# zhazorken/beom

Measured on AMD Instinct MI355X. Metric: cell-layer updates/s, higher is better.
Workload: dtype f64

## Files before the change

### beom_amd/csrc/beom_engine.hip

```cpp
#include <hip/hip_runtime.h>

#include <cmath>
#include <cstdarg>
#include <cstdio>
#include <cstdlib>
#include <cstring>
#include <algorithm>
#include <string>
#include <utility>
#include <vector>

#include "beom_dev.h"
#include "beom_kernels.h"
#include "beom_integrals.h"
#include "beom_series.h"
#include "beom_tracers.h"
#include "beom_tracers_lim.h"
#include "beom_floats.h"
#include "beom_moments.h"
#include "beom_tracer_moments.h"
#include "beom_dense_host.h"

namespace {

// ... 65 lines not shown
    ++A.count;
    ++A.launches;
}

struct beom_engine {
    beom_params P;
    int device = 0;
    hipStream_t stream = nullptr;
    hipStream_t own_stream = nullptr;
    StepTimer *timer = nullptr;
    DevView d{};
    bool dense = false;
    std::vector<void *> allocs;
    const int32_t *slot_of_dev = nullptr;
    bool embedded = false;
    void *stage = nullptr;
    size_t stage_bytes = 0;
    dim3 grid_cells0, grid_cells_layers_flat;
    bool wind = false, bot = false, top = false;
    bool fold_stress = true, fold_static_ok = false;
    bool up_tt = false, up_tb = false, up_tu = false;
    bool last_folded = false;
    bool last_uv_fused = false;
    float *h0r4_dev = nullptr, *out4[3] = {nullptr, nullptr, nullptr};
    float *diag4[3] = {nullptr, nullptr, nullptr};
    double *scan_dev = nullptr;
    int any_u = 0, any_v = 0;
    long long uniform_waves = 0, total_waves = 0;
    bool obc = false;
    bool obc_set = false;
    bool fuse = true;
    bool fuse_uv = true;
    bool lean_visc = true;
    bool visc_all_zero = true;
    bool lean_d2h = true;
    std::vector<int32_t> subc_host, neig_host, dev_index;
    bool lid = false, lid_ready = false;
    int lid_dstep = 2, lid_nring = 0, lid_maxwidth = 1;
    double *lid_ring = nullptr;
    unsigned long long *lid_maxd = nullptr;
    long long lid_sweeps = 0, lid_solves = 0, lid_launches = 0;
    int lid_last = 0;
    int profile_stride = 1;
    bool profile_rotate = false;
    bool split_prod = false;
    bool tile4 = false;
    bool mont_history = true;
    bool mont_keep = false;
    int mont_levels_valid = 0;
    bool hist_stale = false;
    bool last_mont_hist = false;
    bool plain_sweeps = true;
    int last_plain = 0;
    double *integ_part = nullptr, *integ_rows = nullptr;
    int integ_count = 0;
    int32_t *integ_cellmap = nullptr;
    int integ_xper = 0, integ_yper = 0;
    int ntrc = 0;
    int trc_scheme = 1;
    double *trc_q = nullptr, *trc_q_alt = nullptr, *trc_rq[2] = {nullptr, nullptr}, *trc_ctrg = nullptr;
    std::vector<void *> trc_allocs;
    long long nflt = 0;
    bool flt_ready = false;
    double *flt_x = nullptr, *flt_y = nullptr, *flt_k1x = nullptr, *flt_k1y = nullptr, *flt_xs = nullptr, *flt_ys = nullptr;
    int32_t *flt_layer = nullptr, *flt_rej = nullptr;
    unsigned long long *flt_first_dry = nullptr;
    double *flt_rec = nullptr;
    int flt_nrec = 0, flt_stride = 1;
    std::vector<int> flt_rec_tstp;
    long long flt_launches = 0;
    bool cellmap_known = false;
    std::vector<void *> flt_allocs;
    bool flt_band = false;
    FloatBand flt_fb{};
    unsigned long long *flt_in_s = nullptr, *flt_in_n = nullptr;
    int flt_xper = 0, flt_yper = 0;
    double flt_fmm = 0.0;
    long long flt_handovers = 0;
    Accum mom{&kFieldMoments};
    bool mom_by_caller = false;
    int last_tstp = 0;
    Accum tmom{&kTracerMoments};
    int ser_level = 0, ser_stride = 1, ser_nrec = 0, ser_jlo = 1, ser_rows = 0;
    bool ser_by_caller = false;
    double *ser_rec = nullptr;
    std::vector<int> ser_tstp;
    std::vector<void *> ser_allocs;
    char last_err[512] = {0};
};
static int hist_sync(beom_engine *E);
static int leave_mont_history(beom_engine *E);

namespace {

template <class T>
int alloc_plain(beom_engine *E, std::vector<void *> &owner, T **p, size_t n, char *errm, int errm_len, bool zero = true) {
    void *q = nullptr;
    HIP_TRY(hipMalloc(&q, n * sizeof(T)));
    owner.push_back(q);
    if (zero) HIP_TRY(hipMemsetAsync(q, 0, n * sizeof(T), E->stream));
    *p = (T *)q;
    return 0;
}
constexpr size_t kLead = 15;
template <class T>
int alloc_aligned(beom_engine *E, std::vector<void *> &owner, T **p, size_t n, char *errm, int errm_len, bool zero = true) {
// ... 612 lines not shown
    E->ser_tstp.push_back(tstp);
}
template <class CTX>
static bool launch_mont_all(beom_engine *E) {
    const dim3 g = CTX::grid(E->d, 1), b(BEOM_BLOCK);
    switch (E->d.nlay) {
#define CASE_NL(n) case n: hipLaunchKernelGGL((k_update_mont_all<CTX, n>), g, b, 0, E->stream, E->d); return true;
        CASE_NL(1) CASE_NL(2) CASE_NL(3) CASE_NL(4) CASE_NL(5) CASE_NL(6) CASE_NL(7) CASE_NL(8)
#undef CASE_NL
        default: return false;
    }
}
static void launch_mont(beom_engine *E, int ilay) {
    if (ilay == 0) {
        if (E->dense ? launch_mont_all<CellDense>(E) : launch_mont_all<CellGather>(E)) return;
    }
    const int nz = ilay ? 1 : E->d.nlay;
    LAUNCH_CTX(k_update_mont<CellGather>, k_update_mont<CellDense>, nz, E->d, ilay);
}
static bool biharm_tiled(const beom_engine *E) { return E->dense && E->P.svis > 0.0; }
static void launch_visc(beom_engine *E, int ilay) {
    const int nz = ilay ? 1 : E->d.nlay;
    LAUNCH_CTX(k_update_visc<CellGather>, k_update_visc<CellDense>, nz, E->d, ilay);
    if (E->d.svis > 0.0 && biharm_tiled(E) && ilay == 0) {
        if (E->tile4) hipLaunchKernelGGL(k_biharm_tiled<1>, biharm_tiled_grid<1>(E->d), dim3(BEOM_BLOCK), 0, E->stream, E->d);
        else hipLaunchKernelGGL(k_biharm_tiled<2>, biharm_tiled_grid<2>(E->d), dim3(BEOM_BLOCK), 0, E->stream, E->d);
    } else if (E->d.svis > 0.0) {
        const dim3 g = ilay ? E->grid_cells0 : E->grid_cells_layers_flat;
        hipLaunchKernelGGL(k_biharm_lap, g, dim3(BEOM_BLOCK), 0, E->stream, E->d, ilay);
        hipLaunchKernelGGL(k_biharm_flux, g, dim3(BEOM_BLOCK), 0, E->stream, E->d, ilay);
    }
}
template <bool XDIR>
static void launch_uv(beom_engine *E, int ilay, double gene, double ramp, double ctim, bool prod = false) {
    const int nz = ilay ? 1 : E->d.nlay;
    const int copy_hist = ilay ? 1 : 0;
    if (prod) hipLaunchKernelGGL((k_update_uv<CellDense, XDIR, true>), CellDense::grid(E->d, nz), dim3(BEOM_BLOCK), 0, E->stream, E->d, ilay, gene, ramp, ctim, copy_hist);
    else LAUNCH_CTX((k_update_uv<CellGather, XDIR>), (k_update_uv<CellDense, XDIR>), nz, E->d, ilay, gene, ramp, ctim, copy_hist);
    if (!copy_hist) { if (XDIR) rot3(E->d.dmx); else rot3(E->d.dmy); }
}
template <int Q>
static bool raw_mont_visc(beom_engine *E, bool leith, bool plain) {
    const dim3 g = mont_visc_grid<Q>(E->d), b(BEOM_BLOCK);
    switch (E->d.nlay) {
#define MV_GO(n, le, pl) hipLaunchKernelGGL((k_mont_visc<Q, n, le, pl>), g, b, 0, E->stream, E->d)
#define CASE_NL(n) case n: if (plain) { if (leith) MV_GO(n, true, true); else MV_GO(n, false, true); } \
                           else if (leith) MV_GO(n, true, false); else MV_GO(n, false, false); return true;
        CASE_NL(1) CASE_NL(2) CASE_NL(3) CASE_NL(4) CASE_NL(5) CASE_NL(6) CASE_NL(7) CASE_NL(8)
#undef CASE_NL
#undef MV_GO
        default: return false;
    }
}
template <int Q>
static void raw_uv_fused(beom_engine *E, bool first_x, bool prod, bool zv, bool hm, bool plain, double gene, double ramp, double ctim) {
    const dim3 g = uv_fused_grid<Q>(E->d), b(TileGeom<Q>::BLOCK);
    DevView &d = E->d;
#define UV_GO(kern, fx, pr, z) hipLaunchKernelGGL((kern<Q, fx, pr, z>), g, b, 0, E->stream, d, gene, ramp, ctim)
#define UV_PLAIN(fx, z, h) hipLaunchKernelGGL((k_uv_fused<Q, fx, true, z, h, true>), g, b, 0, E->stream, d, gene, ramp, ctim)
#define UV_PICK(fx) do { \
        if (plain) { if (hm) { if (zv) UV_PLAIN(fx, true, true); else UV_PLAIN(fx, false, true); } \
                     else { if (zv) UV_PLAIN(fx, true, false); else UV_PLAIN(fx, false, false); } } \
        else if (hm) { if (zv) hipLaunchKernelGGL((k_uv_fused<Q, fx, true, true, true>), g, b, 0, E->stream, d, gene, ramp, ctim); \
                       else hipLaunchKernelGGL((k_uv_fused<Q, fx, true, false, true>), g, b, 0, E->stream, d, gene, ramp, ctim); } \
        else if (d.stress_fold) { if (zv) UV_GO(k_uv_fused_sf, fx, true, true); else if (prod) UV_GO(k_uv_fused_sf, fx, true, false); else UV_GO(k_uv_fused_sf, fx, false, false); } \
        else { if (zv) UV_GO(k_uv_fused, fx, true, true); else if (prod) UV_GO(k_uv_fused, fx, true, false); else UV_GO(k_uv_fused, fx, false, false); } \
    } while (0)
    if (first_x) UV_PICK(true); else UV_PICK(false);
#undef UV_PICK
#undef UV_PLAIN
#undef UV_GO
}
static bool launch_mont_visc(beom_engine *E, bool uv_fused_follows, bool leith, bool keep_visc) {
    E->d.lean_d2h = uv_fused_follows && E->lean_d2h && !E->d.keep_diag;
    E->d.keep_visc = keep_visc;
    E->d.zero_visc = !leith && uv_fused_follows && E->lean_visc && E->visc_all_zero && E->P.dvis == 0.0 && E->P.bvis == 0.0 &&
                     !E->d.keep_diag;
    const bool plain = E->plain_sweeps && E->d.ocrp == 0.0 && !(E->d.rgld >= 0.5) && !E->d.has_hto && !E->d.keep_diag && !E->d.keep_visc;
    const bool ok = E->tile4 ? raw_mont_visc<1>(E, leith, plain) : raw_mont_visc<2>(E, leith, plain);
    if (ok && plain) E->last_plain |= 2;
    return ok;
}
static void uv_fused_swap(beom_engine *E, bool first_x, bool hm = false) {
    DevView &d = E->d;
    swp(d.u, d.u_alt); swp(d.v, d.v_alt);
    if (first_x) swp(d.h_v, d.hv_alt); else swp(d.h_u, d.hu_alt);
    if (hm) { E->hist_stale = true; return; }
    if (first_x) { rot4(d.dmx); rot3(d.dmy); }
    else         { rot4(d.dmy); rot3(d.dmx); }
}
static void launch_uv_fused(beom_engine *E, bool first_x, bool prod, double gene, double ramp, double ctim,
                            bool swap = true, bool hm = false) {
    const bool zv = prod && E->d.zero_visc;
    const DevView &d = E->d;
    const bool plain = E->plain_sweeps && prod && !d.stress_fold && !d.has_nudg && !d.has_tide && !d.has_stress && !d.has_bodf &&
                       !(d.rgld >= 0.5) && d.svis == 0.0;
    if (plain) E->last_plain |= 1;
    if (E->tile4) raw_uv_fused<1>(E, first_x, prod, zv, hm, plain, gene, ramp, ctim);
    else raw_uv_fused<2>(E, first_x, prod, zv, hm, plain, gene, ramp, ctim);
    if (swap) uv_fused_swap(E, first_x, hm);
}
static bool can_fuse(const beom_engine *E, int n_3d, bool first3) {
    const int nl = E->d.nlay;
    if (!(E->dense && E->fuse && nl <= 8) || E->P.svis > 0.0) return false;
    (void)n_3d;
    if (E->P.dvis > 1.e-3) return true;
    return !first3;
}
static void launch_lid_fluxes(beom_engine *E, bool first3) {
    if (first3) { launch_rebuild(E); return; }
    const dim3 g((unsigned)((E->d.ncell + BEOM_BLOCK - 1) / BEOM_BLOCK), (unsigned)E->d.nlay, 1);
    hipLaunchKernelGGL(k_rgld_upstream_fluxes, g, dim3(BEOM_BLOCK), 0, E->stream, E->d);
}
static void launch_lid_h_epilogue(beom_engine *E) {
    hipLaunchKernelGGL(k_rgld_h_epilogue, dim3((unsigned)((E->d.ncell + BEOM_BLOCK - 1) / BEOM_BLOCK)), dim3(BEOM_BLOCK), 0, E->stream, E->d);
}
static int lid_solve(beom_engine *E) {
    DevView &d = E->d;
    const int maxiters = 1000;
    const double pi_tol = 1.e-5;
    const int R = E->lid_nring, D = E->lid_dstep, nlev = d.sor_ndiag;
    const size_t bytes = (size_t)d.n1 * sizeof(double);
    if (hipMemcpyAsync(E->lid_ring, d.pi_s, bytes, hipMemcpyDeviceToDevice, E->stream) != hipSuccess) return -1;
    int s0 = 1, batch = std::min(R - 1, std::max(16, E->lid_last * 5 / 4 + 8)), chosen = 0;
    unsigned long long maxd[kLidBatch];
    while (!chosen) {
        const int nb = std::min(batch, maxiters - s0 + 1);
        if (hipMemsetAsync(E->lid_maxd, 0, nb * sizeof(unsigned long long), E->stream) != hipSuccess) return -1;
        const dim3 g((unsigned)((E->lid_maxwidth + BEOM_BLOCK - 1) / BEOM_BLOCK), (unsigned)nb, 1);
        const int tend = nlev - 1 + (nb - 1) * D;
        for (int t = 0; t <= tend; ++t)
            hipLaunchKernelGGL(k_rgld_gs_front, g, dim3(BEOM_BLOCK), 0, E->stream, d, E->lid_ring, R, s0, t, D, E->lid_maxd);
        E->lid_launches += tend + 1;
// ... 64 lines not shown
    s.fused_uv = E->dense && E->fuse_uv;
    return s;
}

static bool stress_folds(const beom_engine *E, const StepScalars &s) {
    return E->fold_stress && E->fold_static_ok && s.fused_uv && s.stress && !s.first3 && s.n_3d == 1 && !E->d.keep_diag &&
           (E->wind || !E->up_tt) && (E->bot || !E->up_tb) && (E->top || !E->up_tu);
}

static StepTimer *begin_step(beom_engine *E, int tstp, const StepScalars &s) {
    StepTimer *T = (E->timer && tstp % E->timer->stride == 0) ? E->timer : nullptr;
    if (T) { T->st = E->stream; T->step(tstp); }
    E->d.stress_fold = stress_folds(E, s) ? 1 : 0;
    E->last_folded = E->d.stress_fold != 0;
    return T;
}
template <class F>
static void timed(StepTimer *T, int c, F &&f) {
    if (T) T->begin(c);
    f();
    if (T) T->end();
}

static bool step_front(beom_engine *E, const StepScalars &s, StepTimer *T) {
    if (s.stress && !E->d.stress_fold) launch_stress(E);
    if (E->lid) launch_lid_fluxes(E, s.first3);
    else if (s.first3) launch_rebuild(E);
    if (E->ntrc > 0) timed(T, 7, [&] { launch_tracers(E, s.gene, s.ramp, s.ctim); });
    timed(T, 0, [&] {
        launch_h(E, s.gene, s.ramp, s.ctim);
        if (E->lid) launch_lid_h_epilogue(E);
    });
    const bool leith = E->P.dvis > 1.e-3 && s.upst;
    bool prod = false;
    timed(T, s.fused ? 5 : 1, [&] {
        prod = s.fused && launch_mont_visc(E, s.fused_uv, leith, leith && s.n_3d > 1);
        if (!prod) launch_mont(E, 0);
    });
    if (!prod && (s.first3 || leith || E->P.svis > 0.0)) timed(T, 2, [&] { launch_visc(E, 0); });
    return prod;
}

static bool mont_hist_step(const beom_engine *E, const StepScalars &s) {
    return E->mont_history && E->mont_keep && s.fused && s.fused_uv && s.gene != 0.0 && !stress_folds(E, s) &&
           E->mont_levels_valid >= 3;
}

static void one_step(beom_engine *E, int tstp, const StepScalars &s, int flt = -1) {
    if (flt >= 0 && (flt & 1)) launch_floats(E, 1, nullptr);
    const bool hm = mont_hist_step(E, s);
    if (!hm) (void)hist_sync(E);
    rotate_mont(E);
    StepTimer *T = begin_step(E, tstp, s);
    E->last_plain = 0;
    const bool prod = step_front(E, s, T);
    const bool u_first = tstp % 2 == 0;
    E->last_uv_fused = s.fused_uv;
    E->last_mont_hist = hm;
    if (E->mont_keep) E->mont_levels_valid = std::min(E->mont_levels_valid + 1, 3);
    if (s.fused_uv) timed(T, 6, [&] { launch_uv_fused(E, u_first, prod, s.gene, s.ramp, s.ctim, true, hm && prod); });
    else
        for (const bool x : {u_first, !u_first})
            timed(T, x ? 3 : 4, [&] {
                if (x) launch_uv<true>(E, 0, s.gene, s.ramp, s.ctim, prod);
                else launch_uv<false>(E, 0, s.gene, s.ramp, s.ctim, prod);
            });
    if (E->obc) {
        const dim3 g((unsigned)((E->d.nseg + BEOM_BLOCK - 1) / BEOM_BLOCK), (unsigned)E->d.nlay, 1);
        hipLaunchKernelGGL(k_no_gradient_obc, g, dim3(BEOM_BLOCK), 0, E->stream, E->d, 0);
        hipLaunchKernelGGL(k_no_gradient_obc, g, dim3(BEOM_BLOCK), 0, E->stream, E->d, 1);
    }
    if (E->lid) { launch_lid_fluxes(E, s.first3); launch_lid_pressure(E); }
    E->d.stress_fold = 0;
    if (flt >= 0) launch_floats_after(E, tstp, !(flt & 2));
    E->last_tstp = tstp;
    if (!E->mom_by_caller && accum_due(E->mom, tstp)) launch_moments(E, tstp);
    if (!E->mom_by_caller && accum_due(E->tmom, tstp)) launch_tracer_moments(E, tstp);
    if (!E->ser_by_caller && series_due(E, tstp)) launch_series(E, tstp);
}

template <bool PACK>
static int rows_copy(beom_handle E, int jlo, int nrows, void *dbuf, int jlo2, void *dbuf2) {
    if (!E || !dbuf || jlo < 1 || nrows < 1 || jlo + nrows - 1 > E->d.M) return -3;
    if (dbuf2 && (jlo2 < 1 || jlo2 + nrows - 1 > E->d.M)) return -3;
    if (hipSetDevice(E->device) != hipSuccess) return -9;
    const long long total = 5ll * E->d.nlay * nrows * E->d.L;
    hipLaunchKernelGGL((k_rows_copy<PACK>), dim3((unsigned)((total + BEOM_BLOCK - 1) / BEOM_BLOCK), dbuf2 ? 2u : 1u), dim3(BEOM_BLOCK),
                       0, E->stream, E->d, jlo, nrows, (double *)dbuf, jlo2, (double *)dbuf2);
    if (E->ntrc > 0) {
        const long long tq = (long long)E->ntrc * E->d.nlay * nrows * E->d.L;
        hipLaunchKernelGGL((k_rows_copy_q<PACK>), dim3((unsigned)((tq + BEOM_BLOCK - 1) / BEOM_BLOCK), dbuf2 ? 2u : 1u), dim3(BEOM_BLOCK),
                           0, E->stream, E->d, E->trc_q, E->ntrc, jlo, nrows, (double *)dbuf + total, jlo2, dbuf2 ? (double *)dbuf2 + total : nullptr);
    }
    return hipGetLastError() == hipSuccess ? 0 : -10;
}
extern "C" {

int beom_step(beom_handle E, int tstp_first, int nsteps, double tres, double dtd8, double dt_r,
              double rsta, int n_3d, char *errm, int errm_len) {
    if (!E) { set_err(errm, errm_len, "null handle"); return -1; }
    if (tstp_first < 1 || nsteps < 0 || n_3d < 1) { set_err(errm, errm_len, "beom_step: bad arguments"); return -3; }
    if (E->P.flag_nudging && E->P.mcbc < 0.5 && !E->obc && !E->obc_set) { set_err(errm, errm_len, "beom_step: mcbc = 0 with nudging needs beom_set_open_boundaries (no_gradient_obc, private_mod.f95:2613-2679)"); return -6; }
    if (E->lid && !E->lid_ready) { set_err(errm, errm_len, "beom_step: rgld = 1 needs beom_set_rigid_lid (the Poisson operators Ow, Os, Osum_ and the lid pressure, private_mod.f95:505-563)"); return -6; }
    const bool flt = E->nflt > 0 && !E->flt_band;
    if (flt && !E->flt_ready) { set_err(errm, errm_len, "beom_step: the handle's %lld floats have no positions yet (beom_upload_floats)", E->nflt); return -3; }
    if (flt && E->flt_nrec > 0) {
        long long due = 0;
// ... 38 lines not shown
int beom_profile_stop(beom_handle E, double *ms, int *launches, char *errm, int errm_len) {
    if (!E || !ms || !launches) { set_err(errm, errm_len, "null argument"); return -1; }
    if (!E->timer) { set_err(errm, errm_len, "beom_profile_stop without beom_profile_start"); return -3; }
    HIP_TRY(hipSetDevice(E->device));
    HIP_TRY(hipStreamSynchronize(E->stream));
    StepTimer &T = *E->timer;
    for (int c = 0; c < 8; ++c) { ms[c] = 0.0; launches[c] = 0; }
    for (size_t k = 0; k < T.cls.size(); ++k) {
        float t = 0.f;
        (void)hipEventElapsedTime(&t, T.ev[2 * k], T.ev[2 * k + 1]);
        ms[T.cls[k]] += (double)t;
        launches[T.cls[k]] += 1;
    }
    for (hipEvent_t ev : T.ev) (void)hipEventDestroy(ev);
    delete E->timer;
    E->timer = nullptr;
    HIP_TRY(hipGetLastError());
    return 0;
}

int beom_profile_steps(beom_handle E, int tstp_first, int nsteps, double tres, double dtd8, double dt_r,
                       double rsta, int n_3d, double *ms, int *launches, char *errm, int errm_len) {
    int rc = beom_profile_start(E);
    if (rc) { set_err(errm, errm_len, "null handle"); return rc; }
    rc = beom_step(E, tstp_first, nsteps, tres, dtd8, dt_r, rsta, n_3d, errm, errm_len);
    if (rc) return rc;
    return beom_profile_stop(E, ms, launches, errm, errm_len);
}

static void set_rows(DevView &d, int n, int lo0, int hi0, int lo1 = 1, int hi1 = 0) {
    d.nstrip = n; d.jlo0 = lo0; d.jhi0 = hi0; d.jlo1 = lo1; d.jhi1 = hi1;
}
constexpr int kEdgeRows = 8;

int beom_step_phase(beom_handle E, int tstp, double tres, double dtd8, double dt_r, double rsta, int n_3d,
                    int phase, char *errm, int errm_len) {
    if (!E) { set_err(errm, errm_len, "null handle"); return -1; }
    HIP_TRY(hipSetDevice(E->device));
    DevView &d = E->d;
    if (E->P.flag_nudging && E->P.mcbc < 0.5 && !E->obc && !E->obc_set) { set_err(errm, errm_len, "beom_step_phase: mcbc = 0 with nudging needs beom_set_open_boundaries (no_gradient_obc, private_mod.f95:2613-2679)"); return -6; }
    const StepScalars s = step_scalars(E, tstp, tres, dtd8, dt_r, rsta, n_3d);
    const bool south = d.slab && d.joff > 0, north = d.slab && d.joff + d.M < d.Mg;
    if (!s.fused_uv || !(south || north) || d.M < 4 * kEdgeRows || phase < 1 || phase > 3 || E->obc || E->lid || E->P.svis > 0.0) {
        set_err(errm, errm_len, "beom_step_phase: split step not available for this step/configuration");
        return -20;
    }
    const int M = d.M;
    const bool u_first = tstp % 2 == 0;
    if (leave_mont_history(E)) { set_err(errm, errm_len, "beom_step_phase: the history arrays could not be brought up to date"); return -10; }
    StepTimer *T = begin_step(E, tstp, s);
    E->last_uv_fused = true;
    E->last_mont_hist = false;
    if (phase == 1) {
        E->last_plain = 0;
        E->split_prod = step_front(E, s, T);
    } else if (phase == 2) {
        if (south && north) set_rows(d, 2, 1, kEdgeRows, M - kEdgeRows + 1, M);
        else if (south) set_rows(d, 1, 1, kEdgeRows);
        else set_rows(d, 1, M - kEdgeRows + 1, M);
        timed(T, 6, [&] { launch_uv_fused(E, u_first, E->split_prod, s.gene, s.ramp, s.ctim, false); });
    } else {
        set_rows(d, 1, south ? kEdgeRows + 1 : 1, north ? M - kEdgeRows : M);
        timed(T, 6, [&] { launch_uv_fused(E, u_first, E->split_prod, s.gene, s.ramp, s.ctim, true); });
    }
    set_rows(d, 1, 1, M);
    d.stress_fold = 0;
    E->last_tstp = tstp;
    HIP_TRY(hipGetLastError());
    return 0;
}

int beom_pack_rows(beom_handle E, int jlo, int nrows, void *dbuf) { return rows_copy<true>(E, jlo, nrows, dbuf, 0, nullptr); }
int beom_unpack_rows(beom_handle E, int jlo, int nrows, const void *dbuf) { return rows_copy<false>(E, jlo, nrows, const_cast<void *>(dbuf), 0, nullptr); }
int beom_pack_rows2(beom_handle E, int nrows, int jlo_a, void *dbuf_a, int jlo_b, void *dbuf_b) {
    return rows_copy<true>(E, jlo_a, nrows, dbuf_a, jlo_b, dbuf_b);
}
int beom_unpack_rows2(beom_handle E, int nrows, int jlo_a, const void *dbuf_a, int jlo_b, const void *dbuf_b) {
    return rows_copy<false>(E, jlo_a, nrows, const_cast<void *>(dbuf_a), jlo_b, const_cast<void *>(dbuf_b));
}

int beom_download_outputs(beom_handle E, const float *h0r4, float *eta, float *u4, float *v4,
                          double *minmax, int *thin_layer, char *errm, int errm_len) {
    if (!E) { set_err(errm, errm_len, "null handle"); return -1; }
    HIP_TRY(hipSetDevice(E->device));
    DevView &d = E->d;
    const size_t n = (size_t)d.ndeg * d.nlay;
    if (!E->h0r4_dev) {
        if (!h0r4) { set_err(errm, errm_len, "beom_download_outputs: h_0 (real*4) needed on the first call"); return -3; }
        HIP_TRY(hipMalloc((void **)&E->h0r4_dev, n * sizeof(float)));
        E->allocs.push_back(E->h0r4_dev);
        for (int q = 0; q < 3; ++q) { HIP_TRY(hipMalloc((void **)&E->out4[q], n * sizeof(float))); E->allocs.push_back(E->out4[q]); }
        const size_t nb = (size_t)E->grid_cells0.x;
        HIP_TRY(hipMalloc((void **)&E->scan_dev, nb * d.nlay * 7 * sizeof(double)));
        E->allocs.push_back(E->scan_dev);
    }
    if (h0r4) HIP_TRY(hipMemcpyAsync(E->h0r4_dev, h0r4, n * sizeof(float), hipMemcpyHostToDevice, E->stream));
    const unsigned gx = (unsigned)((d.ncell + BEOM_BLOCK - 1) / BEOM_BLOCK);
    if (eta || u4 || v4) {
        hipLaunchKernelGGL(k_out_convert, dim3(gx), dim3(BEOM_BLOCK), 0, E->stream, d, E->h0r4_dev,
                           eta ? E->out4[0] : nullptr, u4 ? E->out4[1] : nullptr, v4 ? E->out4[2] : nullptr);
        float *host[3] = {eta, u4, v4};
        for (int q = 0; q < 3; ++q)
            if (host[q]) HIP_TRY(hipMemcpyAsync(host[q], E->out4[q], n * sizeof(float), hipMemcpyDeviceToHost, E->stream));
    }
    if (minmax || thin_layer) {
        const size_t nb = (size_t)E->grid_cells0.x;
        hipLaunchKernelGGL(k_out_scan, E->grid_cells0, dim3(BEOM_BLOCK), 0, E->stream, d, E->any_u, E->any_v, E->scan_dev);
// ... 598 lines not shown
        return 0;
    }
    auto S = [&](int is, int col) { return segm[(size_t)is + (size_t)nseg * (col - 1)]; };
    for (int pass = 0; pass < 2; ++pass) {
        std::vector<long long> wr, rd;
        for (int is = 0; is < nseg; ++is) {
            const bool ns = S(is, 5) == 1, ew = S(is, 4) == 1;
            const int comp = pass == 0 ? (ns ? 0 : (ew ? 1 : -1)) : (ns ? 1 : (ew ? 0 : -1));
            if (comp < 0) continue;
            const int ip = pass == 0 ? S(is, 10) : S(is, 1), in = pass == 0 ? S(is, 16) : S(is, 13);
            if (ip == -1) continue;
            if (ip < 1 || ip > E->d.ndeg || in < 0 || in > E->d.ndeg) { set_err(errm, errm_len, "beom_set_open_boundaries: index out of range"); return -3; }
            wr.push_back(2ll * ip + comp);
            rd.push_back(2ll * in + comp);
        }
        std::vector<long long> w2 = wr;
        std::sort(w2.begin(), w2.end());
        if (std::adjacent_find(w2.begin(), w2.end()) != w2.end()) { set_err(errm, errm_len, "beom_set_open_boundaries: two segments update the same point (serial order would matter)"); return -7; }
        for (long long r : rd)
            if (std::binary_search(w2.begin(), w2.end(), r)) { set_err(errm, errm_len, "beom_set_open_boundaries: a segment reads a point another segment updates in the same pass (serial order would matter)"); return -7; }
    }
    std::vector<int32_t> sg(segm, segm + (size_t)nseg * 18);
    if (E->embedded) {
        for (int col : {1, 7, 10, 13, 16})
            for (int is = 0; is < nseg; ++is) {
                int32_t &q = sg[(size_t)is + (size_t)nseg * (col - 1)];
                if (q > 0) { if ((size_t)q >= E->dev_index.size()) { set_err(errm, errm_len, "beom_set_open_boundaries: index out of range"); return -3; } q = E->dev_index[(size_t)q]; }
            }
    } else if (E->d.P)
        for (int col : {1, 7, 10, 13, 16})
            for (int is = 0; is < nseg; ++is) {
                int32_t &q = sg[(size_t)is + (size_t)nseg * (col - 1)];
                if (q > 0) q = (int32_t)(1 + (long long)((q - 1) / E->d.L) * E->d.P + (q - 1) % E->d.L);
            }
    int32_t *dev = nullptr;
    HIP_TRY(hipMalloc((void **)&dev, (size_t)nseg * 18 * sizeof(int32_t)));
    E->allocs.push_back(dev);
    HIP_TRY(hipMemcpy(dev, sg.data(), (size_t)nseg * 18 * sizeof(int32_t), hipMemcpyHostToDevice));
    E->d.segm = dev;
    E->d.nseg = nseg;
    E->obc = E->P.flag_nudging && E->P.mcbc < 0.5;
    E->obc_set = true;
    return 0;
}

int beom_info(beom_handle E, const char *what) {
    if (!E || !what) return -1;
    if (!strcmp(what, "stress_folded")) return E->last_folded ? 1 : 0;
    if (!strcmp(what, "tile_rows")) return E->dense ? (E->tile4 ? 4 : 8) : 0;
    if (!strcmp(what, "biharm_tiled")) return biharm_tiled(E) ? 1 : 0;
    if (!strcmp(what, "uv_fused")) return E->last_uv_fused ? 1 : 0;
    if (!strcmp(what, "mont_history")) return E->last_mont_hist ? 1 : 0;
    if (!strcmp(what, "plain_sweeps")) return E->last_plain;
    if (!strcmp(what, "vel_targets_zero")) return E->d.vel_targets_zero;
    if (!strcmp(what, "tracers")) return E->ntrc;
    if (!strcmp(what, "tracer_scheme")) return E->trc_scheme;
    if (!strcmp(what, "floats")) return (int)std::min<long long>(E->nflt, 2000000000ll);
    if (!strcmp(what, "float_records")) return (int)E->flt_rec_tstp.size();
    if (!strcmp(what, "float_launches")) return (int)std::min<long long>(E->flt_launches, 2000000000ll);
    if (!strcmp(what, "float_handovers")) return (int)std::min<long long>(E->flt_handovers, 2000000000ll);
    if (!strcmp(what, "tracer_moments")) return E->tmom.level;
    if (!strcmp(what, "tracer_moment_samples")) return (int)std::min<long long>(E->tmom.count, 2000000000ll);
    if (!strcmp(what, "tracer_moment_launches")) return (int)std::min<long long>(E->tmom.launches, 2000000000ll);
    if (!strcmp(what, "series")) return E->ser_level;
    if (!strcmp(what, "series_records")) return (int)E->ser_tstp.size();
    if (!strcmp(what, "moments")) return E->mom.level;
    if (!strcmp(what, "moment_samples")) return (int)std::min<long long>(E->mom.count, 2000000000ll);
    if (!strcmp(what, "moment_launches")) return (int)std::min<long long>(E->mom.launches, 2000000000ll);
    if (!strcmp(what, "lid_sweeps")) return (int)std::min<long long>(E->lid_sweeps, 2000000000ll);
    if (!strcmp(what, "lid_solves")) return (int)std::min<long long>(E->lid_solves, 2000000000ll);
    if (!strcmp(what, "lid_launches")) return (int)std::min<long long>(E->lid_launches, 2000000000ll);
    if (!strcmp(what, "lid_sweep_distance")) return E->lid_dstep;
    return -3;
}

int beom_set_option(beom_handle E, const char *name, int value) {
    if (!E || !name) return -1;
    if (!strncmp(name, "fuse", 4) && hist_sync(E)) return -10;
    if (!strcmp(name, "fuse")) { E->fuse = value != 0; E->fuse_uv = value != 0; }
    else if (!strcmp(name, "fuse_mont_visc")) E->fuse = value != 0 && !E->lid;
    else if (!strcmp(name, "fuse_uv")) E->fuse_uv = value != 0 && !E->lid;
    else if (!strcmp(name, "keep_diag")) E->d.keep_diag = value != 0;
    else if (!strcmp(name, "fold_stress")) E->fold_stress = value != 0;
    else if (!strcmp(name, "profile_stride")) E->profile_stride = value > 0 ? value : 1;
    else if (!strcmp(name, "profile_rotate")) E->profile_rotate = value != 0;
    else if (!strcmp(name, "lean_d2h")) E->lean_d2h = value != 0;
    else if (!strcmp(name, "lean_visc")) E->lean_visc = value != 0;
    else if (!strcmp(name, "mont_history")) E->mont_history = value != 0;
    else if (!strcmp(name, "plain_sweeps")) E->plain_sweeps = value != 0;
    else if (!strcmp(name, "moments_by_caller")) E->mom_by_caller = value != 0;
    else return -3;
    return 0;
}

int beom_set_stream(beom_handle E, void *hip_stream, int use_own) {
    if (!E) return -1;
    E->stream = use_own ? E->own_stream : (hipStream_t)hip_stream;
    return 0;
}

int beom_is_dense(beom_handle E) { return (E && E->dense) ? (E->embedded ? 2 : 1) : 0; }

int beom_device_field(beom_handle E, const char *name, void **dptr, int64_t *stride_layer,
                      int64_t *stride_row, int64_t *row0_offset) {
    if (!E || !name || !dptr) return -1;
    const DevView &d = E->d;
// ... 16 lines not shown
```

### beom_amd/csrc/beom_kernels.h

```cpp
#pragma once

#define LL(a, ip, il) (a)[(long long)(ip) + d.n1 * (long long)((il) - 1)]
#define FNUD_(ip, il, iv) d.fnud[(long long)(ip) + d.n1 * ((long long)((il) - 1) + (long long)d.nlay * ((iv) - 1))]
#define FNUDV_(ip, il, iv) d.fnud_vel[(long long)(ip) + d.n1 * ((long long)((il) - 1) + (long long)d.nlay * ((iv) - 2))]
#define NUDG_(ip, iv) d.nudg[(long long)(ip) + d.n1 * ((iv) - 1)]
#define TIDE_(m, ip, iv) d.tide[((m) - 1) + 2 * ((long long)(ip) + d.n1 * ((iv) - 1))]
#define T3_(a, ip, id, il) (a)[(long long)(ip) + d.n1 * ((long long)((id) - 1) + 2 * (long long)((il) - 1))]

__device__ __forceinline__ double powi_dev(double x, int n) {
    double r = x;
    for (int q = 1; q < n; ++q) r = r * x;
    return r;
}

template <class C>
__device__ __forceinline__ void body_rebuild_fluxes(const C &c, const DevView &d) {
    const int ipnt = c.ipnt, ilay = blockIdx.y + 1;
    const int c5 = c.template nb<5>(), c7 = c.template nb<7>();
    const double h0 = LL(d.hlay, ipnt, ilay);
    LL(d.h_u, ipnt, ilay) = LL(d.u, ipnt, ilay) * (h0 + LL(d.hlay, c5, ilay)) / (1.0 + c.mk_u());
    LL(d.h_v, ipnt, ilay) = LL(d.v, ipnt, ilay) * (h0 + LL(d.hlay, c7, ilay)) / (1.0 + c.mk_v());
}
template <class CTX>
__global__ __launch_bounds__(BEOM_BLOCK) void k_rebuild_fluxes(DevView d) {
// ... 368 lines not shown
#pragma unroll
            for (int m = 0; m < l; ++m) mpot = mpot - (d.rhon[l] - d.rhon[m]) * i_rn * hown[m][q];
            if (PLAIN || d.rgld < 0.5) mpot = hcol[q] - h_th[q] + mpot;
            LL(d.mont, ipnt, ilay) = mpot + 0.25 * d.uadv * i_gr
                                          * (u_ri * u_ri + u_le * u_le + v_to * v_to + v_bo * v_bo);
            const double hE = s_hh[buf][r][cx + 1], hW = s_hh[buf][r][cx - 1], hN = s_hh[buf][r + 1][cx],
                         hS = s_hh[buf][r - 1][cx], h6 = s_hh[buf][r - 1][cx - 1];
            if (wr_d2h) {
                double d2x = (hE + hW - h0 * 2.0) * mk1 * mk5 * mkn;
                double d2y = (hN + hS - h0 * 2.0) * mk3 * mk7 * mkn;
                if (!PLAIN && d.ocrp > 0.5) {
                    if (hE < 2.0 * hs_8 || hW < 2.0 * hs_8 || h0 < 2.0 * hs_8) d2x = 0.0;
                    if (hN < 2.0 * hs_8 || hS < 2.0 * hs_8 || h0 < 2.0 * hs_8) d2y = 0.0;
                }
                LL(d.d2hx, ipnt, ilay) = d2x;
                LL(d.d2hy, ipnt, ilay) = d2y;
            }
            const double have = h0 + hW + h6 + hS;
            LL(d.pvor, ipnt, ilay) = (fcor[q] + rv[q] * d.uadv) * mkpi * (mkn + mk5 + mk6 + mk7) / have;
            const double r_bl = rv[q], d_cc = dv[q];
            double vcc, vll;
            if (LEITH) {
                const double r_br = s_rv[buf][r][cx + 1], r_tr = s_rv[buf][r + 1][cx + 1],
                             r_tl = s_rv[buf][r + 1][cx], rbll = s_rv[buf][r][cx - 1], rbbl = s_rv[buf][r - 1][cx];
                const double d_ri = s_dv[buf][r][cx + 1], d_to = s_dv[buf][r + 1][cx],
                             d_le = s_dv[buf][r][cx - 1], d_bl = s_dv[buf][r - 1][cx - 1], d_bo = s_dv[buf][r - 1][cx];
                double a = (r_br - r_bl) * (r_br - r_bl) + (r_bl - rbll) * (r_bl - rbll)
                         + (r_tl - r_bl) * (r_tl - r_bl) + (r_bl - rbbl) * (r_bl - rbbl)
                         + (d_cc - d_le) * (d_cc - d_le) + (d_bo - d_bl) * (d_bo - d_bl)
                         + (d_cc - d_bo) * (d_cc - d_bo) + (d_le - d_bl) * (d_le - d_bl);
                vll = sqrt(a) * d.dvis * d.dl * d.dl + d.bvis;
                double b = (r_br - r_bl) * (r_br - r_bl) + (r_tr - r_tl) * (r_tr - r_tl)
                         + (r_tl - r_bl) * (r_tl - r_bl) + (r_tr - r_br) * (r_tr - r_br)
                         + (d_ri - d_cc) * (d_ri - d_cc) + (d_cc - d_le) * (d_cc - d_le)
                         + (d_to - d_cc) * (d_to - d_cc) + (d_cc - d_bo) * (d_cc - d_bo);
                vcc = sqrt(b) * d.dvis * d.dl * d.dl + d.bvis;
            } else {
                vcc = vcc0[q]; vll = vll0[q];
            }
            if (LEITH || wr_prod) {
                LL(d.pcd, ipnt, ilay) = vcc * d_cc;
                LL(d.qlr, ipnt, ilay) = vll * r_bl;
            }
            if (!PLAIN && d.keep_diag) {
                LL(d.rvor, ipnt, ilay) = r_bl; LL(d.dive, ipnt, ilay) = d_cc;
                if (LEITH) { LL(d.v_cc, ipnt, ilay) = vcc; LL(d.v_ll, ipnt, ilay) = vll; }
            } else if (!PLAIN && LEITH && d.keep_visc) {
                LL(d.v_cc, ipnt, ilay) = vcc; LL(d.v_ll, ipnt, ilay) = vll;
            }
        }
    }
}

template <int Q, int NL, bool LEITH = true, bool PLAIN = false>
__global__ __launch_bounds__(BEOM_BLOCK) __attribute__((amdgpu_waves_per_eu(3))) void k_mont_visc(DevView d) {
    using G = TileGeom<Q>;
    __shared__ double s_rv[LEITH ? 2 : 1][LEITH ? G::MV_LDY : 1][LEITH ? G::MV_LDX : 1];
    __shared__ double s_dv[LEITH ? 2 : 1][LEITH ? G::MV_LDY : 1][LEITH ? G::MV_LDX : 1];
    __shared__ double s_hh[2][G::MV_LDY][G::MV_LDX];
    const TileMap tm(d, G::TX, G::TY);
    int ty, ch;
    if (!tm.locate(blockIdx.x, ty, ch)) return;
    const int x0 = ch * G::TX + 1, y0 = ty * G::TY + 1;
    const bool interior = x0 - 1 >= 2 && x0 + G::TX <= d.L - 2 && y0 - 1 >= 2 && y0 + G::TY <= d.M - 2
                          && y0 - 1 + d.joff >= 2 && y0 + G::TY + d.joff <= d.Mg - 2 && tile_regular(d, x0, y0, G::TY);
    const int uy0 = ((y0 - 1) / G::TY) * G::TY + 1;
    bool deep = x0 - 1 - G::TX >= 2 && x0 + 2 * G::TX <= d.L - 2 && uy0 - 1 - G::TY >= 2 && uy0 + 2 * G::TY <= d.M - 2
                && uy0 - 1 - G::TY + d.joff >= 2 && uy0 + 2 * G::TY + d.joff <= d.Mg - 2;
    if (deep && d.embedded)
        for (int dy = -1; dy <= 1; ++dy)
            for (int dx = -1; dx <= 1; ++dx) deep = deep && tile_regular(d, x0 + dx * G::TX, uy0 + dy * G::TY, G::TY);
    const bool wr_d2h = !(d.lean_d2h && deep);
    const bool wr_prod = !(d.zero_visc && deep);
    if (interior) body_mont_visc<Q, NL, true, LEITH, PLAIN>(d, x0, y0, wr_d2h, wr_prod, (double (*)[G::MV_LDY][G::MV_LDX])s_rv, (double (*)[G::MV_LDY][G::MV_LDX])s_dv, s_hh);
    else body_mont_visc<Q, NL, false, LEITH, PLAIN>(d, x0, y0, wr_d2h, wr_prod, (double (*)[G::MV_LDY][G::MV_LDX])s_rv, (double (*)[G::MV_LDY][G::MV_LDX])s_dv, s_hh);
}
template <int Q>
static inline dim3 mont_visc_grid(const DevView &d) { return dim3(TileMap(d, TileGeom<Q>::TX, TileGeom<Q>::TY).blocks(), 1, 1); }

template <class C>
__device__ __forceinline__ void body_update_visc(const C &c, const DevView &d, int ilay_only) {
    const int ipnt = c.ipnt;
    const int ilay = ilay_only ? ilay_only : (int)blockIdx.y + 1;
    const int c1 = c.template nb<1>(), c2 = c.template nb<2>(), c3 = c.template nb<3>(),
              c5 = c.template nb<5>(), c6 = c.template nb<6>(), c7 = c.template nb<7>();
    const double r_bl = LL(d.rvor, ipnt, ilay), r_br = LL(d.rvor, c1, ilay), r_tr = LL(d.rvor, c2, ilay),
                 r_tl = LL(d.rvor, c3, ilay), rbll = LL(d.rvor, c5, ilay), rbbl = LL(d.rvor, c7, ilay);
    const double d_cc = LL(d.dive, ipnt, ilay), d_ri = LL(d.dive, c1, ilay), d_to = LL(d.dive, c3, ilay),
                 d_le = LL(d.dive, c5, ilay), d_bl = LL(d.dive, c6, ilay), d_bo = LL(d.dive, c7, ilay);
    double a = (r_br - r_bl) * (r_br - r_bl) + (r_bl - rbll) * (r_bl - rbll)
             + (r_tl - r_bl) * (r_tl - r_bl) + (r_bl - rbbl) * (r_bl - rbbl)
             + (d_cc - d_le) * (d_cc - d_le) + (d_bo - d_bl) * (d_bo - d_bl)
             + (d_cc - d_bo) * (d_cc - d_bo) + (d_le - d_bl) * (d_le - d_bl);
    LL(d.v_ll, ipnt, ilay) = sqrt(a) * d.dvis * d.dl * d.dl + d.bvis;
    double b = (r_br - r_bl) * (r_br - r_bl) + (r_tr - r_tl) * (r_tr - r_tl)
             + (r_tl - r_bl) * (r_tl - r_bl) + (r_tr - r_br) * (r_tr - r_br)
             + (d_ri - d_cc) * (d_ri - d_cc) + (d_cc - d_le) * (d_cc - d_le)
             + (d_to - d_cc) * (d_to - d_cc) + (d_cc - d_bo) * (d_cc - d_bo);
    LL(d.v_cc, ipnt, ilay) = sqrt(b) * d.dvis * d.dl * d.dl + d.bvis;
}
template <class CTX>
__global__ __launch_bounds__(BEOM_BLOCK) void k_update_visc(DevView d, int ilay_only) {
    CTX c;
    if (!c.init(d)) return;
    if (c.wave_is_interior()) body_update_visc(c.as_interior(), d, ilay_only);
    else body_update_visc(c, d, ilay_only);
}

struct UVio {
    const double *vel_in; double *vel_out;
    double *hp_out;
    const double *dm0, *dm1, *dm2;
    double *dm_out;
};

template <int Q>
using UVstage = double[TileGeom<Q>::SROWS][TileGeom<Q>::SLDX];
template <int Q>
using UVhstage = double[TileGeom<Q>::HROWS][TileGeom<Q>::HLDX];

struct ShGlobal {
    const DevView &d; int ipnt, cb, ca, ilay;
    __device__ __forceinline__ double hlay_s() const { return LL(d.hlay, ipnt, ilay); }
    __device__ __forceinline__ double hlay_b() const { return LL(d.hlay, cb, ilay); }
    __device__ __forceinline__ double mont_s() const { return LL(d.mont, ipnt, ilay); }
    __device__ __forceinline__ double mont_b() const { return LL(d.mont, cb, ilay); }
    __device__ __forceinline__ double pvor_s() const { return LL(d.pvor, ipnt, ilay); }
// ... 1232 lines not shown
```

Before: 20.86 billion.

## Raise mont_visc occupancy and split boundary tiles into two half-height passes

```diff
diff --git a/beom_amd/csrc/beom_engine.hip b/beom_amd/csrc/beom_engine.hip
--- a/beom_amd/csrc/beom_engine.hip
+++ b/beom_amd/csrc/beom_engine.hip
@@ -141,6 +141,7 @@
     bool last_mont_hist = false;
     bool plain_sweeps = true;
     int last_plain = 0;
+    int last_mv = -1;
     double *integ_part = nullptr, *integ_rows = nullptr;
     int integ_count = 0;
     int32_t *integ_cellmap = nullptr;
@@ -859,6 +860,32 @@
         default: return false;
     }
 }
+static inline int mont_visc_key(bool tile4, int nlay, bool leith, bool plain) { return (((tile4 ? 0 : 1) * 8 + nlay - 1) * 2 + (leith ? 1 : 0)) * 2 + (plain ? 1 : 0); }
+template <int Q>
+static int raw_mont_visc_blocks(int nlay, bool leith, bool plain) {
+    int nb = 0;
+    hipError_t r = hipErrorInvalidValue;
+    switch (nlay) {
+#define MV_OCC(n, le, pl) r = hipOccupancyMaxActiveBlocksPerMultiprocessor(&nb, k_mont_visc<Q, n, le, pl>, BEOM_BLOCK, 0)
+#define CASE_NL(n) case n: if (plain) { if (leith) MV_OCC(n, true, true); else MV_OCC(n, false, true); } \
+                           else if (leith) MV_OCC(n, true, false); else MV_OCC(n, false, false); break;
+        CASE_NL(1) CASE_NL(2) CASE_NL(3) CASE_NL(4) CASE_NL(5) CASE_NL(6) CASE_NL(7) CASE_NL(8)
+#undef CASE_NL
+#undef MV_OCC
+        default: break;
+    }
+    return r == hipSuccess ? nb : -9;
+}
+static int mont_visc_blocks_per_cu(int key) {
+    static int kept[64];
+    if (key < 0 || key >= 64) return 0;
+    if (kept[key] == 0) {
+        const bool plain = key & 1, leith = (key >> 1) & 1;
+        const int nlay = ((key >> 2) & 7) + 1;
+        kept[key] = (key >> 5) ? raw_mont_visc_blocks<2>(nlay, leith, plain) : raw_mont_visc_blocks<1>(nlay, leith, plain);
+    }
+    return kept[key];
+}
 template <int Q>
 static void raw_uv_fused(beom_engine *E, bool first_x, bool prod, bool zv, bool hm, bool plain, double gene, double ramp, double ctim) {
     const dim3 g = uv_fused_grid<Q>(E->d), b(TileGeom<Q>::BLOCK);
@@ -886,6 +913,7 @@
     const bool plain = E->plain_sweeps && E->d.ocrp == 0.0 && !(E->d.rgld >= 0.5) && !E->d.has_hto && !E->d.keep_diag && !E->d.keep_visc;
     const bool ok = E->tile4 ? raw_mont_visc<1>(E, leith, plain) : raw_mont_visc<2>(E, leith, plain);
     if (ok && plain) E->last_plain |= 2;
+    if (ok) E->last_mv = mont_visc_key(E->tile4, E->d.nlay, leith, plain);
     return ok;
 }
 static void uv_fused_swap(beom_engine *E, bool first_x, bool hm = false) {
@@ -1056,7 +1084,7 @@
     if (!hm) (void)hist_sync(E);
     rotate_mont(E);
     StepTimer *T = begin_step(E, tstp, s);
-    E->last_plain = 0;
+    E->last_plain = 0; E->last_mv = -1;
     const bool prod = step_front(E, s, T);
     const bool u_first = tstp % 2 == 0;
     E->last_uv_fused = s.fused_uv;
@@ -1201,7 +1229,7 @@
     E->last_uv_fused = true;
     E->last_mont_hist = false;
     if (phase == 1) {
-        E->last_plain = 0;
+        E->last_plain = 0; E->last_mv = -1;
         E->split_prod = step_front(E, s, T);
     } else if (phase == 2) {
         if (south && north) set_rows(d, 2, 1, kEdgeRows, M - kEdgeRows + 1, M);
@@ -1906,6 +1934,11 @@
     if (!strcmp(what, "uv_fused")) return E->last_uv_fused ? 1 : 0;
     if (!strcmp(what, "mont_history")) return E->last_mont_hist ? 1 : 0;
     if (!strcmp(what, "plain_sweeps")) return E->last_plain;
+    if (!strcmp(what, "mont_visc_blocks_per_cu")) {
+        if (E->last_mv < 0) return 0;
+        if (hipSetDevice(E->device) != hipSuccess) return -9;
+        return mont_visc_blocks_per_cu(E->last_mv);
+    }
     if (!strcmp(what, "vel_targets_zero")) return E->d.vel_targets_zero;
     if (!strcmp(what, "tracers")) return E->ntrc;
     if (!strcmp(what, "tracer_scheme")) return E->trc_scheme;
diff --git a/beom_amd/csrc/beom_kernels.h b/beom_amd/csrc/beom_kernels.h
--- a/beom_amd/csrc/beom_kernels.h
+++ b/beom_amd/csrc/beom_kernels.h
@@ -444,9 +444,17 @@
     }
 }
 
+constexpr int mont_visc_waves(int Q, int NL, bool LEITH, bool PLAIN) {
+    if (Q != 2) return 3;
+    if (LEITH && (NL == 8 || (NL == 7 && !PLAIN))) return 3;
+    if (LEITH && PLAIN && NL == 4) return 3;
+    return 4;
+}
 template <int Q, int NL, bool LEITH = true, bool PLAIN = false>
-__global__ __launch_bounds__(BEOM_BLOCK) __attribute__((amdgpu_waves_per_eu(3))) void k_mont_visc(DevView d) {
+__global__ __launch_bounds__(BEOM_BLOCK) __attribute__((amdgpu_waves_per_eu(mont_visc_waves(Q, NL, LEITH, PLAIN)))) void k_mont_visc(DevView d) {
     using G = TileGeom<Q>;
+    using H = TileGeom<1>;
+    static_assert(H::MV_LDY <= G::MV_LDY && H::MV_LDX == G::MV_LDX && 2 * H::TY >= G::TY, "two 64 x 4 passes cover the tile, their stage lies inside its stage");
     __shared__ double s_rv[LEITH ? 2 : 1][LEITH ? G::MV_LDY : 1][LEITH ? G::MV_LDX : 1];
     __shared__ double s_dv[LEITH ? 2 : 1][LEITH ? G::MV_LDY : 1][LEITH ? G::MV_LDX : 1];
     __shared__ double s_hh[2][G::MV_LDY][G::MV_LDX];
@@ -465,6 +473,15 @@
     const bool wr_d2h = !(d.lean_d2h && deep);
     const bool wr_prod = !(d.zero_visc && deep);
     if (interior) body_mont_visc<Q, NL, true, LEITH, PLAIN>(d, x0, y0, wr_d2h, wr_prod, (double (*)[G::MV_LDY][G::MV_LDX])s_rv, (double (*)[G::MV_LDY][G::MV_LDX])s_dv, s_hh);
+    else if (Q == 2) {
+        double (*h_rv)[H::MV_LDY][H::MV_LDX] = (double (*)[H::MV_LDY][H::MV_LDX])s_rv;
+        double (*h_dv)[H::MV_LDY][H::MV_LDX] = (double (*)[H::MV_LDY][H::MV_LDX])s_dv;
+        double (*h_hh)[H::MV_LDY][H::MV_LDX] = (double (*)[H::MV_LDY][H::MV_LDX])s_hh;
+        body_mont_visc<1, NL, false, LEITH, PLAIN>(d, x0, y0, wr_d2h, wr_prod, h_rv, h_dv, h_hh);
+        if (y0 + H::TY > d.M) return;
+        __syncthreads();
+        body_mont_visc<1, NL, false, LEITH, PLAIN>(d, x0, y0 + H::TY, wr_d2h, wr_prod, h_rv, h_dv, h_hh);
+    }
     else body_mont_visc<Q, NL, false, LEITH, PLAIN>(d, x0, y0, wr_d2h, wr_prod, (double (*)[G::MV_LDY][G::MV_LDX])s_rv, (double (*)[G::MV_LDY][G::MV_LDX])s_dv, s_hh);
 }
 template <int Q>
```

Result: no change. 20.83 billion (-0.2%).
